# GAP-LAB-CUHK-SZ/REC-MV

Hardware: AMD Instinct MI355X
Metric: optimiser iters/sec, female-3-casual-like 512x512 (synthetic frames) (higher is better)
Workload: dtype f32

## Files before the change

rec-mv_amd/csrc/gemm_f32.hip:

```cpp
#include <mutex>
#include <unordered_map>
#include <type_traits>
#include <vector>
#include "common.h"
#ifdef RECMV_LIBM_SOFTPLUS
#define RECMV_EXPF(x) expf(x)
#define RECMV_LOG1PF(t) log1pf(t)
#else
#define RECMV_EXPF(x) __expf(x)
#define RECMV_LOG1PF(t) __logf(1.f + (t))
#endif

#include <algorithm>

namespace recmv {
namespace {

typedef float f32x16 __attribute__((ext_vector_type(16)));
typedef float f32x2 __attribute__((ext_vector_type(2)));
typedef __bf16 bf16x2 __attribute__((ext_vector_type(2)));
typedef __bf16 bf16x8 __attribute__((ext_vector_type(8)));
typedef unsigned int u32x4 __attribute__((ext_vector_type(4)));

struct Pieces {
  bf16x8 h, m, l;
};
__device__ __forceinline__ unsigned pack_bf16(float a, float b) {
#ifdef RECMV_SPLIT_INT
  unsigned ua = __float_as_uint(a), ub = __float_as_uint(b);
  ua += 0x7fffu + ((ua >> 16) & 1u);
  ub += 0x7fffu + ((ub >> 16) & 1u);
  return (ua >> 16) | (ub & 0xffff0000u);
#else
// ... 292 lines not shown
    }
    if (kt + 1 < nk) lstore(buf ^ 1);
    __syncthreads();
  }

  constexpr int LDC = TBN + 4;
  float* Cs = smem;
#pragma unroll
  for (int mi = 0; mi < T; ++mi)
#pragma unroll
    for (int ni = 0; ni < T; ++ni)
#pragma unroll
      for (int r = 0; r < 16; ++r) {
        const int row = wm * WT + mi * 32 + (r & 3) + 8 * (r >> 2) + 4 * (lane >> 5);
        const int col = wn * WT + ni * 32 + (lane & 31);
        Cs[row * LDC + col] = acc[mi][ni][r];
      }
  __syncthreads();
  switch (act) {
    case RECMV_ACT_RELU:
      nt_epilogue<T, RECMV_ACT_RELU>(Cs, bias, C, ldc, M, N, m0, n0, act_param, out_scale, c_vec, AMUL ? AMul{nullptr, 0, 0, 0.f, 1.f, 1.f} : am);
      break;
    case RECMV_ACT_SOFTPLUS:
      nt_epilogue<T, RECMV_ACT_SOFTPLUS>(Cs, bias, C, ldc, M, N, m0, n0, act_param, out_scale, c_vec, AMUL ? AMul{nullptr, 0, 0, 0.f, 1.f, 1.f} : am);
      break;
    case RECMV_ACT_TANH:
      nt_epilogue<T, RECMV_ACT_TANH>(Cs, bias, C, ldc, M, N, m0, n0, act_param, out_scale, c_vec, AMUL ? AMul{nullptr, 0, 0, 0.f, 1.f, 1.f} : am);
      break;
    default:
      nt_epilogue<T, RECMV_ACT_NONE>(Cs, bias, C, ldc, M, N, m0, n0, act_param, out_scale, c_vec, AMUL ? AMul{nullptr, 0, 0, 0.f, 1.f, 1.f} : am);
  }
}

template <bool AMUL, int BKT, bool SINGLE, int MI, int NI>
__global__ __launch_bounds__(kBlk, (MI * NI == 4 ? (BKT <= 16 ? 4 : 3) : 5))
void gemm_nt_occ_kernel(const float* __restrict__ A, int64_t lda, const float* __restrict__ B, int64_t ldb,
                        const float* __restrict__ bias, float* __restrict__ C, int64_t ldc, int M, int N, int K, int act,
                        float act_param, float out_scale, int nbm, int nbn, bool c_vec, AMul am) {
  constexpr int TBM = 64 * MI, TBN = 64 * NI;
  constexpr int LDKT = BKT + 4;
  constexpr int C4R = BKT / 4;
  constexpr int NLA = TBM * C4R / kBlk, NLB = TBN * C4R / kBlk;
  constexpr int NBUF = SINGLE ? 1 : 2;
  extern __shared__ __attribute__((aligned(16))) float smem[];
  float* As = smem;
  float* Bs = smem + NBUF * TBM * LDKT;
  const int tid = threadIdx.x, lane = tid & 63, wave = tid >> 6;
  const int wm = wave >> 1, wn = wave & 1;
  const int64_t logical = xcd_remap(blockIdx.x, (int64_t)nbm * nbn);
  const int tile_m = (int)(logical / nbn), tile_n = (int)(logical % nbn);
  const int m0 = tile_m * TBM, n0 = tile_n * TBN;
  if (am.B2 && m0 >= am.split) {
    B = am.B2;
    bias = am.bias2;
  }
  f32x16 acc[MI][NI];
#pragma unroll
  for (int a = 0; a < MI; ++a)
#pragma unroll
    for (int b = 0; b < NI; ++b)
#pragma unroll
      for (int r = 0; r < 16; ++r) acc[a][b][r] = 0.f;

  float4 ra[NLA], rb[NLB];
  const float* pa[NLA];
  const float* pb[NLB];
  const float* py[NLA];
#pragma unroll
  for (int r = 0; r < NLA; ++r) {
    const int idx = tid + kBlk * r;
    int gm = m0 + idx / C4R;
    gm = gm < M ? gm : M - 1;
    pa[r] = A + (int64_t)gm * lda + (idx % C4R) * 4;
    if (AMUL) py[r] = am.Y + (int64_t)gm * am.ldy + (idx % C4R) * 4;
  }
#pragma unroll
  for (int r = 0; r < NLB; ++r) {
    const int idx = tid + kBlk * r;
    int gn = n0 + idx / C4R;
    gn = gn < N ? gn : N - 1;
    pb[r] = B + (int64_t)gn * ldb + (idx % C4R) * 4;
  }
  auto gload = [&](int k0) {
#pragma unroll
    for (int r = 0; r < NLA; ++r) {
      const bool in = k0 + ((tid + kBlk * r) % C4R) * 4 < K;
      ra[r] = in ? *reinterpret_cast<const float4*>(pa[r] + k0) : make_float4(0, 0, 0, 0);
      if (AMUL && in) ra[r] = amul4(ra[r], *reinterpret_cast<const float4*>(py[r] + k0), am);
    }
#pragma unroll
    for (int r = 0; r < NLB; ++r) {
      const bool in = k0 + ((tid + kBlk * r) % C4R) * 4 < K;
      rb[r] = in ? *reinterpret_cast<const float4*>(pb[r] + k0) : make_float4(0, 0, 0, 0);
    }
  };
  auto lstore = [&](int buf) {
#pragma unroll
    for (int r = 0; r < NLA; ++r) {
      const int idx = tid + kBlk * r;
      *reinterpret_cast<float4*>(As + (buf * TBM + idx / C4R) * LDKT + (idx % C4R) * 4) = ra[r];
    }
#pragma unroll
    for (int r = 0; r < NLB; ++r) {
      const int idx = tid + kBlk * r;
      *reinterpret_cast<float4*>(Bs + (buf * TBN + idx / C4R) * LDKT + (idx % C4R) * 4) = rb[r];
    }
  };

  const int nk = (K + BKT - 1) / BKT;
  gload(0);
  lstore(0);
  __syncthreads();
  const int arow = wm * 32 * MI + (lane & 31), brow = wn * 32 * NI + (lane & 31), khalf = (lane >> 5) * 4;
  for (int kt = 0; kt < nk; ++kt) {
    const int buf = SINGLE ? 0 : (kt & 1);
    if (kt + 1 < nk) gload((kt + 1) * BKT);
    const float* as = As + (buf * TBM + arow) * LDKT + khalf;
    const float* bs = Bs + (buf * TBN + brow) * LDKT + khalf;
#pragma unroll
    for (int kk = 0; kk < BKT / 8; ++kk) {
      float4 a[MI], b[NI];
#pragma unroll
      for (int i = 0; i < MI; ++i) a[i] = *reinterpret_cast<const float4*>(as + i * 32 * LDKT + kk * 8);
#pragma unroll
      for (int i = 0; i < NI; ++i) b[i] = *reinterpret_cast<const float4*>(bs + i * 32 * LDKT + kk * 8);
// ... 14 lines not shown

  constexpr int HR = 32 * MI, LDC = TBN + 4;
  float* Cs = smem;
  const AMul em = AMUL ? AMul{nullptr, 0, 0, 0.f, 1.f, 1.f} : am;
#pragma unroll 1
  for (int h = 0; h < 2; ++h) {
    if (h) __syncthreads();
    if (wm == h) {
#pragma unroll
      for (int mi = 0; mi < MI; ++mi)
#pragma unroll
        for (int ni = 0; ni < NI; ++ni)
#pragma unroll
          for (int r = 0; r < 16; ++r) {
            const int row = mi * 32 + (r & 3) + 8 * (r >> 2) + 4 * (lane >> 5);
            const int col = wn * 32 * NI + ni * 32 + (lane & 31);
            Cs[row * LDC + col] = acc[mi][ni][r];
          }
    }
    __syncthreads();
    const int mh = m0 + HR * h;
    switch (act) {
      case RECMV_ACT_RELU:
        nt_epilogue_rows<HR, TBN, RECMV_ACT_RELU>(Cs, bias, C, ldc, M, N, mh, n0, act_param, out_scale, c_vec, em);
        break;
      case RECMV_ACT_SOFTPLUS:
        nt_epilogue_rows<HR, TBN, RECMV_ACT_SOFTPLUS>(Cs, bias, C, ldc, M, N, mh, n0, act_param, out_scale, c_vec, em);
        break;
      case RECMV_ACT_TANH:
        nt_epilogue_rows<HR, TBN, RECMV_ACT_TANH>(Cs, bias, C, ldc, M, N, mh, n0, act_param, out_scale, c_vec, em);
        break;
      default:
        nt_epilogue_rows<HR, TBN, RECMV_ACT_NONE>(Cs, bias, C, ldc, M, N, mh, n0, act_param, out_scale, c_vec, em);
    }
  }
}

__device__ __forceinline__ int b3_off(int row, int chunk) { return row * 64 + ((chunk ^ ((row >> 2) & 3)) << 4); }

struct B3Pre {
  const char* planes;
  const char* planes2;
  int64_t plane_bytes, plane_bytes2;
  int Kp;
};

template <int T, bool AMUL, bool PRE>
__global__ __launch_bounds__(kBlk, 2) void gemm_nt_b3_kernel(const float* __restrict__ A, int64_t lda,
                                                             const float* __restrict__ B, int64_t ldb,
                                                             const float* __restrict__ bias, float* __restrict__ C,
                                                             int64_t ldc, int M, int N, int K, int act,
                                                             float act_param, float out_scale, int nbm, int nbn,
                                                             bool c_vec, AMul am, B3Pre pre) {
  constexpr int TBM = 64 * T, TBN = 64 * T, WT = 32 * T;
  constexpr int NI = TBM * 4 / kBlk;
  constexpr int PLANE = TBM * 64;
  constexpr int NSET = 1;
  extern __shared__ __attribute__((aligned(16))) float smem[];
  char* As = reinterpret_cast<char*>(smem);
  char* Bs = As + 3 * PLANE;
  const int tid = threadIdx.x, lane = tid & 63, wave = tid >> 6;
  const int wm = wave >> 1, wn = wave & 1;
  const int64_t logical = xcd_remap(blockIdx.x, (int64_t)nbm * nbn);
  const int tile_m = (int)(logical / nbn), tile_n = (int)(logical % nbn);
  const int m0 = tile_m * TBM, n0 = tile_n * TBN;
  const char* planes = pre.planes;
// ... 533 lines not shown
    } else {
    const float* as = As + (buf * BK + kh) * LDM + acol;
    const float* bs = Bs + (buf * BK + kh) * LDM + bcol;
#pragma unroll
    for (int k2 = 0; k2 < BK / 2; ++k2) {
      const float a0 = as[k2 * 2 * LDM], a1 = as[k2 * 2 * LDM + 32];
      const float b0 = bs[k2 * 2 * LDM], b1 = bs[k2 * 2 * LDM + 32];
      acc[0][0] = __builtin_amdgcn_mfma_f32_32x32x2f32(a0, b0, acc[0][0], 0, 0, 0);
      acc[0][1] = __builtin_amdgcn_mfma_f32_32x32x2f32(a0, b1, acc[0][1], 0, 0, 0);
      acc[1][0] = __builtin_amdgcn_mfma_f32_32x32x2f32(a1, b0, acc[1][0], 0, 0, 0);
      acc[1][1] = __builtin_amdgcn_mfma_f32_32x32x2f32(a1, b1, acc[1][1], 0, 0, 0);
    }
    }
    if (kt + 1 < nk) lstore(buf ^ 1);
    __syncthreads();
  }

  float* Ps = P + (int64_t)split * M * N;
#pragma unroll
  for (int ni = 0; ni < 2; ++ni) {
    const int gn = n0 + wn * 64 + ni * 32 + (lane & 31);
    if (gn >= N) continue;
#pragma unroll
    for (int mi = 0; mi < 2; ++mi) {
#pragma unroll
      for (int r = 0; r < 16; ++r) {
        const int gm = m0 + wm * 64 + mi * 32 + (r & 3) + 8 * (r >> 2) + 4 * (lane >> 5);
        if (gm < M) Ps[(int64_t)gm * N + gn] = acc[mi][ni][r];
      }
    }
  }
}

template <int BKT>
__global__ __launch_bounds__(kBlk, 4) void gemm_tn_occ_kernel(const float* __restrict__ A, int64_t lda,
                                                              const float* __restrict__ B, int64_t ldb,
                                                              float* __restrict__ P, int M, int N, int64_t K, int nbm,
                                                              int nbn, int64_t kchunk) {
  constexpr int NLD = BKT * 32 / kBlk;
  extern __shared__ __attribute__((aligned(16))) float smem[];
  float* As = smem;
  float* Bs = smem + BKT * LDM;
  const int tid = threadIdx.x, lane = tid & 63, wave = tid >> 6;
  const int wm = wave >> 1, wn = wave & 1;
  const int tiles = nbm * nbn;
  int split = blockIdx.x / tiles, tile = blockIdx.x % tiles;
  const int splits = gridDim.x / tiles;
  if (splits % kNumXCD == 0) {
    const int x = blockIdx.x % kNumXCD, j = blockIdx.x / kNumXCD;
    split = x + kNumXCD * (j / tiles);
    tile = j % tiles;
  }
  const int tile_m = tile / nbn, tile_n = tile % nbn;
  const int m0 = tile_m * BM, n0 = tile_n * BN;
  const int64_t kbeg = (int64_t)split * kchunk;
  int64_t kend = kbeg + kchunk;
  if (kend > K) kend = K;

  f32x16 acc[2][2];
#pragma unroll
  for (int a = 0; a < 2; ++a)
#pragma unroll
    for (int b = 0; b < 2; ++b)
#pragma unroll
      for (int r = 0; r < 16; ++r) acc[a][b][r] = 0.f;

  float4 ra[NLD], rb[NLD];
  const bool whole_mn = m0 + BM <= M && n0 + BN <= N;
  auto gload = [&](int64_t k0) {
    const bool whole = whole_mn && k0 + BKT <= kend;
#pragma unroll
    for (int r = 0; r < NLD; ++r) {
      const int idx = tid + kBlk * r;
      const int krow = idx >> 5, c4 = idx & 31;
      const int64_t k = k0 + krow;
      const int cm = m0 + c4 * 4, cn = n0 + c4 * 4;
      if (whole) {
        ra[r] = *reinterpret_cast<const float4*>(A + k * lda + cm);
        rb[r] = *reinterpret_cast<const float4*>(B + k * ldb + cn);
      } else {
        const bool kin = k < kend, ain = kin && cm < M, bin = kin && cn < N;
        const int64_t kc = kin ? k : kend - 1;
        float4 a = *reinterpret_cast<const float4*>(A + kc * lda + (cm < M ? cm : (M - 1) & ~3));
        float4 b = *reinterpret_cast<const float4*>(B + kc * ldb + (cn < N ? cn : (N - 1) & ~3));
        ra[r] = make_float4(ain ? a.x : 0.f, ain ? a.y : 0.f, ain ? a.z : 0.f, ain ? a.w : 0.f);
        rb[r] = make_float4(bin ? b.x : 0.f, bin ? b.y : 0.f, bin ? b.z : 0.f, bin ? b.w : 0.f);
      }
    }
  };
  auto lstore = [&]() {
#pragma unroll
    for (int r = 0; r < NLD; ++r) {
      const int idx = tid + kBlk * r;
      const int krow = idx >> 5, c4 = idx & 31;
      *reinterpret_cast<float4*>(As + krow * LDM + c4 * 4) = ra[r];
      *reinterpret_cast<float4*>(Bs + krow * LDM + c4 * 4) = rb[r];
    }
  };

  const int nk = (int)((kend - kbeg + BKT - 1) / BKT);
  if (nk > 0) {
    gload(kbeg);
    lstore();
  }
  __syncthreads();
  const int acol = wm * 64 + (lane & 31), bcol = wn * 64 + (lane & 31), kh = lane >> 5;
  const float* as = As + kh * LDM + acol;
  const float* bs = Bs + kh * LDM + bcol;
  for (int kt = 0; kt < nk; ++kt) {
    if (kt + 1 < nk) gload(kbeg + (int64_t)(kt + 1) * BKT);
#pragma unroll
    for (int k2 = 0; k2 < BKT / 2; ++k2) {
      const float a0 = as[k2 * 2 * LDM], a1 = as[k2 * 2 * LDM + 32];
      const float b0 = bs[k2 * 2 * LDM], b1 = bs[k2 * 2 * LDM + 32];
      acc[0][0] = __builtin_amdgcn_mfma_f32_32x32x2f32(a0, b0, acc[0][0], 0, 0, 0);
      acc[0][1] = __builtin_amdgcn_mfma_f32_32x32x2f32(a0, b1, acc[0][1], 0, 0, 0);
      acc[1][0] = __builtin_amdgcn_mfma_f32_32x32x2f32(a1, b0, acc[1][0], 0, 0, 0);
      acc[1][1] = __builtin_amdgcn_mfma_f32_32x32x2f32(a1, b1, acc[1][1], 0, 0, 0);
    }
    __syncthreads();
    if (kt + 1 < nk) lstore();
    __syncthreads();
  }

  float* Ps = P + (int64_t)split * M * N;
#pragma unroll
  for (int ni = 0; ni < 2; ++ni) {
    const int gn = n0 + wn * 64 + ni * 32 + (lane & 31);
    if (gn >= N) continue;
#pragma unroll
    for (int mi = 0; mi < 2; ++mi) {
#pragma unroll
      for (int r = 0; r < 16; ++r) {
        const int gm = m0 + wm * 64 + mi * 32 + (r & 3) + 8 * (r >> 2) + 4 * (lane >> 5);
        if (gm < M) Ps[(int64_t)gm * N + gn] = acc[mi][ni][r];
      }
    }
  }
}

__global__ __launch_bounds__(kBlk) void splitk_reduce_kernel(const float* __restrict__ P, float* __restrict__ C,
                                                             int64_t ldc, int M, int N, int splits) {
  const int64_t total = (int64_t)M * N;
  for (int64_t i = (int64_t)blockIdx.x * kBlk + threadIdx.x; i < total; i += (int64_t)gridDim.x * kBlk) {
    float s = 0.f;
    for (int sp = 0; sp < splits; ++sp) s += P[(int64_t)sp * total + i];
    C[(i / N) * ldc + (i % N)] = s;
  }
}

__global__ __launch_bounds__(kBlk) void splitk_reduce4_kernel(const float4* __restrict__ P, float* __restrict__ C,
                                                              int64_t ldc, int M, int N, int splits) {
  const int64_t total4 = (int64_t)M * N / 4;
  for (int64_t i = (int64_t)blockIdx.x * kBlk + threadIdx.x; i < total4; i += (int64_t)gridDim.x * kBlk) {
    float4 s = make_float4(0.f, 0.f, 0.f, 0.f);
    int sp = 0;
    for (; sp + 8 <= splits; sp += 8) {
      float4 v[8];
#pragma unroll
      for (int u = 0; u < 8; ++u) v[u] = P[(int64_t)(sp + u) * total4 + i];
#pragma unroll
      for (int u = 0; u < 8; ++u) {
        s.x += v[u].x;
        s.y += v[u].y;
        s.z += v[u].z;
        s.w += v[u].w;
      }
    }
    for (; sp < splits; ++sp) {
      const float4 v = P[(int64_t)sp * total4 + i];
      s.x += v.x;
// ... 78 lines not shown
    if (!active) return;
    const double flops = 2.0 * M * N * K;
    r.bytes = 4.0 * (M * K + N * K + M * N);
    if (flops < g_prof.min_flops) {
      std::lock_guard<std::mutex> lk(g_prof.mu);
      g_prof.untimed[variant][0] += 1.0;
      g_prof.untimed[variant][1] += flops;
      active = false;
      return;
    }
    r.variant = variant;
    r.flops = flops;
    r.a = g_prof.get();
    r.b = g_prof.get();
    if (!r.a || !r.b) {
      active = false;
      return;
    }
    (void)hipEventRecord(r.a, s);
  }
  ~ScopedLaunchTimer() {
    if (!active) return;
    (void)hipEventRecord(r.b, s);
    std::lock_guard<std::mutex> lk(g_prof.mu);
    g_prof.recs.push_back(r);
  }
};

inline bool aligned16(const void* p) { return (reinterpret_cast<uintptr_t>(p) & 15) == 0; }

constexpr int kNtLds = (2 * BM * LDK + 2 * BN * LDK) * 4;
constexpr int kTnLds = (4 * BK * LDM) * 4;

bool tn_occ() {
  static const bool v = [] { const char* e = getenv("RECMV_GEMM_OCC"); return !(e && e[0] == '0'); }();
  return v;
}

int tn_splits(int64_t M, int64_t N, int64_t K) {
  const int64_t tiles = ceil_div(M, BM) * ceil_div(N, BN);
  int64_t want = ceil_div((int64_t)kNumCU * 4, tiles);
  const int64_t maxs = ceil_div(K, (int64_t)BK * 4);
  if (want > maxs) want = maxs;
  if (want > 128) want = 128;
  if (want < 1) want = 1;
  return (int)want;
}

}
}

using namespace recmv;

int g_b3_families = 7;
int g_gemm_mode = 0;

template <int T, bool FAST, bool AMUL, bool BF3>
static int launch_nt(const float* A, int64_t lda, const float* B, int64_t ldb, const float* bias, float* C,
                     int64_t ldc, int64_t M, int64_t N, int64_t K, int act, float act_param, float out_scale,
                     bool a_vec, bool b_vec, bool c_vec, const AMul& am, hipStream_t stream) {
  constexpr int lds = kNtLds / (T == 2 ? 1 : 2);
  static bool attr_set = false;
  if (!attr_set) {
    RECMV_HIP_TRY(hipFuncSetAttribute((const void*)gemm_nt_kernel<T, FAST, AMUL, BF3>,
                                      hipFuncAttributeMaxDynamicSharedMemorySize, lds));
    attr_set = true;
  }
  const int nbm = (int)ceil_div(M, 64 * T), nbn = (int)ceil_div(N, 64 * T);
  ScopedLaunchTimer timer((T - 1) + 2 * (FAST ? 1 : 0) + 4 * (AMUL ? 1 : 0), (double)M, (double)N, (double)K, stream);
  hipLaunchKernelGGL((gemm_nt_kernel<T, FAST, AMUL, BF3>), dim3((unsigned)((int64_t)nbm * nbn)), dim3(kBlk), lds, stream, A,
                     lda, B, ldb, bias, C, ldc, (int)M, (int)N, (int)K, act, act_param, out_scale, nbm, nbn, a_vec,
                     b_vec, c_vec, am);
  return check_launch("gemm_nt");
}

template <bool AMUL, int BKT, bool SINGLE, int MI, int NI>
static int launch_nt_occ(const float* A, int64_t lda, const float* B, int64_t ldb, const float* bias, float* C,
                         int64_t ldc, int64_t M, int64_t N, int64_t K, int act, float act_param, float out_scale,
                         bool c_vec, const AMul& am, hipStream_t stream) {
  constexpr int lds_ops = (SINGLE ? 1 : 2) * 64 * (MI + NI) * (BKT + 4) * 4, lds_c = 32 * MI * (64 * NI + 4) * 4;
  constexpr int lds = lds_ops > lds_c ? lds_ops : lds_c;
  const int nbm = (int)ceil_div(M, 64 * MI), nbn = (int)ceil_div(N, 64 * NI);
  ScopedLaunchTimer timer(AMUL ? 11 : (MI == 2 ? 9 : 10), (double)M, (double)N, (double)K, stream);
  hipLaunchKernelGGL((gemm_nt_occ_kernel<AMUL, BKT, SINGLE, MI, NI>), dim3((unsigned)((int64_t)nbm * nbn)), dim3(kBlk), lds,
                     stream, A, lda, B, ldb, bias, C, ldc, (int)M, (int)N, (int)K, act, act_param, out_scale, nbm, nbn, c_vec,
                     am);
  return check_launch("gemm_nt(occ)");
}

struct B3Entry {
  const char* planes;
  int64_t N, K, ldb, Kp;
};
static std::mutex g_b3_mu;
static std::unordered_map<const float*, B3Entry> g_b3;
static bool b3_lookup(const float* B, int64_t N, int64_t K, int64_t ldb, B3Entry* out) {
  std::lock_guard<std::mutex> lock(g_b3_mu);
  auto it = g_b3.find(B);
  if (it == g_b3.end() || it->second.K != K || it->second.ldb != ldb || it->second.N < N) return false;
  *out = it->second;
  return true;
}

template <int T, bool AMUL, bool PRE>
static int launch_nt_b3_as(const float* A, int64_t lda, const float* B, int64_t ldb, const float* bias, float* C, int64_t ldc,
                           int64_t M, int64_t N, int64_t K, int act, float act_param, float out_scale, bool c_vec, const AMul& am,
                           const B3Pre& pre, hipStream_t stream) {
  constexpr int lds_ops = 6 * 64 * T * 64, lds_c = 64 * T * (64 * T + 4) * 4;
  constexpr int lds = lds_ops > lds_c ? lds_ops : lds_c;
  static bool attr_set = false;
  if (!attr_set) {
    RECMV_HIP_TRY(hipFuncSetAttribute((const void*)gemm_nt_b3_kernel<T, AMUL, PRE>,
                                      hipFuncAttributeMaxDynamicSharedMemorySize, lds));
    attr_set = true;
  }
  const int nbm = (int)ceil_div(M, 64 * T), nbn = (int)ceil_div(N, 64 * T);
  ScopedLaunchTimer timer((T - 1) + 2 + 4 * (AMUL ? 1 : 0), (double)M, (double)N, (double)K, stream);
  hipLaunchKernelGGL((gemm_nt_b3_kernel<T, AMUL, PRE>), dim3((unsigned)((int64_t)nbm * nbn)), dim3(kBlk), lds, stream, A, lda,
                     B, ldb, bias, C, ldc, (int)M, (int)N, (int)K, act, act_param, out_scale, nbm, nbn, c_vec, am, pre);
  return check_launch("gemm_nt(b3)");
// ... 6 lines not shown
  B3Entry e, e2;
  if (b3_lookup(B, N, K, ldb, &e) && (!am.B2 || (b3_lookup(am.B2, N, K, ldb, &e2) && e2.Kp == e.Kp))) {
    B3Pre pre = {e.planes, am.B2 ? e2.planes : nullptr, e.N * e.Kp * 2, am.B2 ? e2.N * e2.Kp * 2 : 0, (int)e.Kp};
    return launch_nt_b3_as<T, AMUL, true>(A, lda, B, ldb, bias, C, ldc, M, N, K, act, act_param, out_scale, c_vec, am, pre, stream);
  }
  B3Pre none = {nullptr, nullptr, 0, 0, 0};
  return launch_nt_b3_as<T, AMUL, false>(A, lda, B, ldb, bias, C, ldc, M, N, K, act, act_param, out_scale, c_vec, am, none, stream);
}

constexpr int kNarrowLds = 2 * (64 + 32) * LDK * 4;

template <bool FAST, bool AMUL, bool BF3>
static int launch_nt_narrow(const float* A, int64_t lda, const float* B, int64_t ldb, const float* bias, float* C,
                            int64_t ldc, int64_t M, int64_t N, int64_t K, int act, float act_param, float out_scale,
                            bool a_vec, bool b_vec, bool c_vec, const AMul& am, hipStream_t stream) {
  const int nbm = (int)ceil_div(M, 64), nbn = (int)ceil_div(N, 32);
  ScopedLaunchTimer timer(FAST && !AMUL ? 12 : 13, (double)M, (double)N, (double)K, stream);
  hipLaunchKernelGGL((gemm_nt_narrow_kernel<FAST, AMUL, BF3>), dim3((unsigned)((int64_t)nbm * nbn)), dim3(kBlk),
                     kNarrowLds, stream, A, lda, B, ldb, bias, C, ldc, (int)M, (int)N, (int)K, act, act_param, out_scale,
                     nbm, nbn, a_vec, b_vec, c_vec, am);
  return check_launch("gemm_nt(narrow)");
}

template <bool AMUL>
static int dispatch_nt(const float* A, int64_t lda, const float* B, int64_t ldb, const float* bias, float* C,
                       int64_t ldc, int64_t M, int64_t N, int64_t K, int act, float act_param, float out_scale,
                       const AMul& am, hipStream_t s) {
  const bool a_vec = aligned16(A) && lda % 4 == 0 && (!AMUL || (aligned16(am.Y) && am.ldy % 4 == 0));
  const bool b_vec = aligned16(B) && ldb % 4 == 0 && (!am.B2 || aligned16(am.B2));
  const bool c_vec = aligned16(C) && ldc % 4 == 0;
  const bool fast = a_vec && b_vec && K % 4 == 0 && K > 0;
  const int64_t big_blocks = ceil_div(M, BM) * ceil_div(N, BN);
  const bool bf3_big = g_gemm_mode == 1 && (g_b3_families & 1), bf3_mid = g_gemm_mode == 1 && (g_b3_families & 2);
#define RECMV_NT(TT, FF)                                                                                          \
  ((TT == 2 ? bf3_big : bf3_mid) ? launch_nt<TT, FF, AMUL, true>(A, lda, B, ldb, bias, C, ldc, M, N, K, act, act_param, out_scale, \
                                                    a_vec, b_vec, c_vec, am, s)                                    \
                    : launch_nt<TT, FF, AMUL, false>(A, lda, B, ldb, bias, C, ldc, M, N, K, act, act_param,        \
                                                     out_scale, a_vec, b_vec, c_vec, am, s))
  if (big_blocks >= 2 * kNumCU) {
    if (bf3_big && fast) {
      return launch_nt_b3<2, AMUL>(A, lda, B, ldb, bias, C, ldc, M, N, K, act, act_param, out_scale, c_vec, am, s);
    }
    static const bool occ = [] { const char* e = getenv("RECMV_GEMM_OCC"); return !(e && e[0] == '0'); }();
    if (fast && !bf3_big && occ) {
      if (big_blocks >= 3600)
        return launch_nt_occ<AMUL, 16, true, 2, 2>(A, lda, B, ldb, bias, C, ldc, M, N, K, act, act_param, out_scale, c_vec, am, s);
      return launch_nt_occ<AMUL, 16, true, 1, 2>(A, lda, B, ldb, bias, C, ldc, M, N, K, act, act_param, out_scale, c_vec, am, s);
    }
    return fast ? RECMV_NT(2, true) : RECMV_NT(2, false);
  }
  const int64_t mid_blocks = ceil_div(M, 64) * ceil_div(N, 64);
  if (mid_blocks < (5 * kNumCU) / 2) {
#define RECMV_NTN(FF)                                                                                                  \
  (bf3_mid ? launch_nt_narrow<FF, AMUL, true>(A, lda, B, ldb, bias, C, ldc, M, N, K, act, act_param, out_scale, \
                                                       a_vec, b_vec, c_vec, am, s)                                     \
                    : launch_nt_narrow<FF, AMUL, false>(A, lda, B, ldb, bias, C, ldc, M, N, K, act, act_param,          \
                                                        out_scale, a_vec, b_vec, c_vec, am, s))
    return fast ? RECMV_NTN(true) : RECMV_NTN(false);
#undef RECMV_NTN
  }
  return fast ? RECMV_NT(1, true) : RECMV_NT(1, false);
#undef RECMV_NT
}

extern "C" int recmv_set_gemm_mode(int mode) {
  const int prev = g_gemm_mode;
  if (mode == 0 || mode == 1) g_gemm_mode = mode;
  return prev;
}

extern "C" int recmv_get_gemm_mode(void) { return g_gemm_mode; }

extern "C" int recmv_set_b3_families(int mask) {
  const int prev = g_b3_families;
  if (mask >= 0 && mask <= 7) g_b3_families = mask;
  return prev;
}

extern "C" int64_t recmv_b3_planes_bytes(int64_t N, int64_t K) {
  if (N <= 0 || K <= 0) return 0;
  return 3 * N * (ceil_div(K, (int64_t)BK) * BK) * 2;
// ... 104 lines not shown
                             void* stream) {
  RECMV_REQUIRE(M >= 0 && N >= 0 && K >= 0, "gemm_tn: negative size");
  if (M == 0 || N == 0) return RECMV_OK;
  RECMV_REQUIRE(M < (1 << 20) && N < (1 << 20), "gemm_tn: output too large");
  hipStream_t s = (hipStream_t)stream;
  if (K == 0) {
    RECMV_REQUIRE(C && ldc >= N, "gemm_tn: bad output");
    for (int64_t m = 0; m < M; ++m) RECMV_HIP_TRY(hipMemsetAsync(C + m * ldc, 0, N * 4, s));
    return RECMV_OK;
  }
  RECMV_REQUIRE(A && B && C, "gemm_tn: NULL pointer");
  RECMV_REQUIRE(lda >= M && ldb >= N && ldc >= N, "gemm_tn: leading dimension too small");
  const int splits = tn_splits(M, N, K);
  const int64_t need = (int64_t)splits * M * N * 4;
  if (!workspace || workspace_bytes < need) {
    set_error("gemm_tn: workspace %lld < %lld bytes", (long long)workspace_bytes, (long long)need);
    return RECMV_ERR_WORKSPACE;
  }
  static bool attr_set = false;
  if (!attr_set) {
    RECMV_HIP_TRY(hipFuncSetAttribute((const void*)gemm_tn_kernel<false>, hipFuncAttributeMaxDynamicSharedMemorySize,
                                      kTnLds));
    RECMV_HIP_TRY(hipFuncSetAttribute((const void*)gemm_tn_kernel<true>, hipFuncAttributeMaxDynamicSharedMemorySize,
                                      kTnLds));
    attr_set = true;
  }
  const int nbm = (int)ceil_div(M, BM), nbn = (int)ceil_div(N, BN);
  int64_t kchunk = ceil_div(ceil_div(K, splits), BK) * BK;
  const bool a_vec = aligned16(A) && lda % 4 == 0, b_vec = aligned16(B) && ldb % 4 == 0;
  int rc;
  {
  ScopedLaunchTimer timer(8, (double)M, (double)N, (double)K, s);
  const bool bf3_tn = g_gemm_mode == 1 && (g_b3_families & 4);
  if (!bf3_tn && tn_occ() && a_vec && b_vec && lda >= ((M + 3) & ~3ll) && ldb >= ((N + 3) & ~3ll) && M >= 4 && N >= 4) {
    kchunk = ceil_div(ceil_div(K, splits), 16) * 16;
    hipLaunchKernelGGL(gemm_tn_occ_kernel<16>, dim3((unsigned)(nbm * nbn * splits)), dim3(kBlk), 2 * 16 * LDM * 4, s, A, lda,
                       B, ldb, (float*)workspace, (int)M, (int)N, K, nbm, nbn, kchunk);
  } else if (bf3_tn)
    hipLaunchKernelGGL(gemm_tn_kernel<true>, dim3((unsigned)(nbm * nbn * splits)), dim3(kBlk), kTnLds, s, A, lda, B,
                       ldb, (float*)workspace, (int)M, (int)N, K, nbm, nbn, kchunk, a_vec, b_vec);
  else
    hipLaunchKernelGGL(gemm_tn_kernel<false>, dim3((unsigned)(nbm * nbn * splits)), dim3(kBlk), kTnLds, s, A, lda, B,
                       ldb, (float*)workspace, (int)M, (int)N, K, nbm, nbn, kchunk, a_vec, b_vec);
  rc = check_launch("gemm_tn");
  }
  if (rc) return rc;
  if (N % 4 == 0 && ldc % 4 == 0 && aligned16(C) && aligned16(workspace))
    hipLaunchKernelGGL(splitk_reduce4_kernel, dim3(stream_grid(M * N / 4, kBlk)), dim3(kBlk), 0, s,
                       (const float4*)workspace, C, ldc, (int)M, (int)N, splits);
  else
    hipLaunchKernelGGL(splitk_reduce_kernel, dim3(stream_grid(M * N, kBlk)), dim3(kBlk), 0, s,
                       (const float*)workspace, C, ldc, (int)M, (int)N, splits);
  return check_launch("gemm_tn/reduce");
}

extern "C" int recmv_posenc_forward(const float* x, int64_t ldx, float* out, int64_t ldo, int64_t ldo_fill,
                                    int64_t P, int L, const float* weights_host, float out_scale,
                                    void* stream) {
  RECMV_REQUIRE(P >= 0 && L >= 0 && L <= 16, "posenc: bad size (P=%lld, L=%d)", (long long)P, L);
  if (P == 0) return RECMV_OK;
  RECMV_REQUIRE(x && out, "posenc: NULL pointer");
  RECMV_REQUIRE(ldx >= 3 && ldo >= 3 + 6 * L && ldo_fill <= ldo, "posenc: leading dimension too small");
  hipStream_t s = (hipStream_t)stream;
  PeWeights hw;
  for (int i = 0; i < 32; ++i) hw.w[i] = (weights_host && i < 2 * L) ? weights_host[i] : 1.f;
  hipLaunchKernelGGL(posenc_kernel, dim3(stream_grid(P * (1 + 2 * L), kBlk)), dim3(kBlk), 0, s, x, ldx, out, ldo,
                     ldo_fill, P, L, hw, out_scale);
  return check_launch("posenc");
}

extern "C" int recmv_profile_begin(double min_flops) {
  g_prof.recs.clear();
  for (auto& u : g_prof.untimed) u[0] = u[1] = 0.0;
  g_prof.min_flops = min_flops;
  g_prof.on = true;
  return RECMV_OK;
// ... 82 lines not shown
```

Measured before the change: 10.33.

## Add skinny GEMM routes for thin N, thin K, and unaligned operands

Adds dedicated kernels for NT GEMMs with K<=4 or N<=4 and for TN GEMMs with an output dimension <=4. Also adds an unaligned-operand variant of the occupancy NT and TN kernels that uses dword-aligned vector loads instead of falling back to the generic kernel. The aim is to stop small-dimension and misaligned shapes from wasting large MFMA tiles, and to let them use the faster occupancy paths. These routes are on by default behind environment switches, and a shape-logging helper is added. This adds more template instantiations and new edge-case handling for partial vectors.

```diff
diff --git a/rec-mv_amd/csrc/gemm_f32.hip b/rec-mv_amd/csrc/gemm_f32.hip
--- a/rec-mv_amd/csrc/gemm_f32.hip
+++ b/rec-mv_amd/csrc/gemm_f32.hip
@@ -1,4 +1,5 @@
 #include <mutex>
+#include <string>
 #include <unordered_map>
 #include <type_traits>
 #include <vector>
@@ -357,11 +358,24 @@
   }
 }
 
-template <bool AMUL, int BKT, bool SINGLE, int MI, int NI>
+typedef float f32x4_a4 __attribute__((ext_vector_type(4), aligned(4)));
+__device__ __forceinline__ float4 load4_dword(const float* __restrict__ p, int limit) {
+  if (limit >= 4) {
+    const f32x4_a4 v = *reinterpret_cast<const f32x4_a4*>(p);
+    return make_float4(v.x, v.y, v.z, v.w);
+  }
+  return load4_guard(p, limit, false);
+}
+
+__device__ __forceinline__ float4 keep4(float4 v, int limit) {
+  return make_float4(limit > 0 ? v.x : 0.f, limit > 1 ? v.y : 0.f, limit > 2 ? v.z : 0.f, limit > 3 ? v.w : 0.f);
+}
+
+template <bool AMUL, int BKT, bool SINGLE, int MI, int NI, bool SCAL = false>
 __global__ __launch_bounds__(kBlk, (MI * NI == 4 ? (BKT <= 16 ? 4 : 3) : 5))
 void gemm_nt_occ_kernel(const float* __restrict__ A, int64_t lda, const float* __restrict__ B, int64_t ldb,
                         const float* __restrict__ bias, float* __restrict__ C, int64_t ldc, int M, int N, int K, int act,
-                        float act_param, float out_scale, int nbm, int nbn, bool c_vec, AMul am) {
+                        float act_param, float out_scale, int nbm, int nbn, bool c_vec, AMul am, bool a_vec, bool b_vec) {
   constexpr int TBM = 64 * MI, TBN = 64 * NI;
   constexpr int LDKT = BKT + 4;
   constexpr int C4R = BKT / 4;
@@ -391,6 +405,7 @@
   const float* pa[NLA];
   const float* pb[NLB];
   const float* py[NLA];
+  bool va[NLA], vb[NLB];
 #pragma unroll
   for (int r = 0; r < NLA; ++r) {
     const int idx = tid + kBlk * r;
@@ -398,6 +413,7 @@
     gm = gm < M ? gm : M - 1;
     pa[r] = A + (int64_t)gm * lda + (idx % C4R) * 4;
     if (AMUL) py[r] = am.Y + (int64_t)gm * am.ldy + (idx % C4R) * 4;
+    va[r] = a_vec && gm < M - 1;
   }
 #pragma unroll
   for (int r = 0; r < NLB; ++r) {
@@ -405,17 +421,33 @@
     int gn = n0 + idx / C4R;
     gn = gn < N ? gn : N - 1;
     pb[r] = B + (int64_t)gn * ldb + (idx % C4R) * 4;
+    vb[r] = b_vec && gn < N - 1;
   }
   auto gload = [&](int k0) {
 #pragma unroll
     for (int r = 0; r < NLA; ++r) {
-      const bool in = k0 + ((tid + kBlk * r) % C4R) * 4 < K;
+      const int k = k0 + ((tid + kBlk * r) % C4R) * 4;
+      if (SCAL) {
+        ra[r] = va[r] ? keep4(k < K ? *reinterpret_cast<const float4*>(pa[r] + k0) : make_float4(0, 0, 0, 0), K - k)
+                      : load4_dword(pa[r] + k0, K - k);
+        if (AMUL && k < K)
+          ra[r] = amul4(ra[r], va[r] ? keep4(*reinterpret_cast<const float4*>(py[r] + k0), K - k)
+                                     : load4_dword(py[r] + k0, K - k), am);
+        continue;
+      }
+      const bool in = k < K;
       ra[r] = in ? *reinterpret_cast<const float4*>(pa[r] + k0) : make_float4(0, 0, 0, 0);
       if (AMUL && in) ra[r] = amul4(ra[r], *reinterpret_cast<const float4*>(py[r] + k0), am);
     }
 #pragma unroll
     for (int r = 0; r < NLB; ++r) {
-      const bool in = k0 + ((tid + kBlk * r) % C4R) * 4 < K;
+      const int k = k0 + ((tid + kBlk * r) % C4R) * 4;
+      if (SCAL) {
+        rb[r] = vb[r] ? keep4(k < K ? *reinterpret_cast<const float4*>(pb[r] + k0) : make_float4(0, 0, 0, 0), K - k)
+                      : load4_dword(pb[r] + k0, K - k);
+        continue;
+      }
+      const bool in = k < K;
       rb[r] = in ? *reinterpret_cast<const float4*>(pb[r] + k0) : make_float4(0, 0, 0, 0);
     }
   };
@@ -496,6 +528,163 @@
         break;
       default:
         nt_epilogue_rows<HR, TBN, RECMV_ACT_NONE>(Cs, bias, C, ldc, M, N, mh, n0, act_param, out_scale, c_vec, em);
+    }
+  }
+}
+
+__device__ __forceinline__ float apply_act_rt(float z, int act, float p, float inv_p) {
+  switch (act) {
+    case RECMV_ACT_RELU: return apply_act<RECMV_ACT_RELU>(z, p, inv_p);
+    case RECMV_ACT_SOFTPLUS: return apply_act<RECMV_ACT_SOFTPLUS>(z, p, inv_p);
+    case RECMV_ACT_TANH: return apply_act<RECMV_ACT_TANH>(z, p, inv_p);
+    default: return z;
+  }
+}
+
+constexpr int kThinRows = 128;
+template <int NN, bool VEC>
+__global__ __launch_bounds__(kThinRows) void gemm_nt_thin_n_kernel(const float* __restrict__ A, int64_t lda,
+                                                                   const float* __restrict__ B, int64_t ldb,
+                                                                   const float* __restrict__ bias, float* __restrict__ C,
+                                                                   int64_t ldc, int M, int K, int act, float act_param,
+                                                                   float out_scale, bool halves, AMul am) {
+  __shared__ __attribute__((aligned(16))) float As[kThinRows * LDK];
+  __shared__ __attribute__((aligned(16))) float Bs[4 * LDK];
+  const int tid = threadIdx.x;
+  const int m0 = blockIdx.x * kThinRows;
+  if (am.B2 && m0 >= am.split) {
+    B = am.B2;
+    bias = am.bias2;
+  }
+  constexpr int NLD = kThinRows * 8 / kThinRows;
+  float4 ra[NLD];
+  float rb;
+  const float* pa[NLD];
+#pragma unroll
+  for (int r = 0; r < NLD; ++r) {
+    const int idx = tid + kThinRows * r;
+    int gm = m0 + (idx >> 3);
+    gm = gm < M ? gm : M - 1;
+    pa[r] = A + (int64_t)gm * lda + (idx & 7) * 4;
+  }
+  const int bn = tid >> 5, bk = tid & 31;
+  auto gload = [&](int k0) {
+#pragma unroll
+    for (int r = 0; r < NLD; ++r) {
+      const int k = k0 + ((tid + kThinRows * r) & 7) * 4;
+      if (VEC)
+        ra[r] = k < K ? *reinterpret_cast<const float4*>(pa[r] + k0) : make_float4(0, 0, 0, 0);
+      else
+        ra[r] = load4_dword(pa[r] + k0, K - k);
+    }
+    rb = (bn < NN && k0 + bk < K) ? B[(int64_t)bn * ldb + k0 + bk] : 0.f;
+  };
+  auto lstore = [&]() {
+#pragma unroll
+    for (int r = 0; r < NLD; ++r) {
+      const int idx = tid + kThinRows * r;
+      *reinterpret_cast<float4*>(As + (idx >> 3) * LDK + (idx & 7) * 4) = ra[r];
+    }
+    Bs[bn * LDK + bk] = rb;
+  };
+  float acc[2][NN];
+#pragma unroll
+  for (int n = 0; n < NN; ++n) acc[0][n] = acc[1][n] = 0.f;
+  const int nk = (K + BK - 1) / BK;
+  gload(0);
+  lstore();
+  __syncthreads();
+  const float* as = As + tid * LDK;
+  for (int kt = 0; kt < nk; ++kt) {
+    if (kt + 1 < nk) gload((kt + 1) * BK);
+#pragma unroll
+    for (int kk = 0; kk < BK / 8; ++kk) {
+      const float4 a0 = *reinterpret_cast<const float4*>(as + kk * 8);
+      const float4 a1 = *reinterpret_cast<const float4*>(as + kk * 8 + 4);
+#pragma unroll
+      for (int n = 0; n < NN; ++n) {
+        const float4 b0 = *reinterpret_cast<const float4*>(Bs + n * LDK + kk * 8);
+        const float4 b1 = *reinterpret_cast<const float4*>(Bs + n * LDK + kk * 8 + 4);
+        const int h = (halves && kk >= BK / 16) ? 1 : 0;
+        float s = acc[h][n];
+        s = fmaf(a0.x, b0.x, s);
+        s = fmaf(a1.x, b1.x, s);
+        s = fmaf(a0.y, b0.y, s);
+        s = fmaf(a1.y, b1.y, s);
+        s = fmaf(a0.z, b0.z, s);
+        s = fmaf(a1.z, b1.z, s);
+        s = fmaf(a0.w, b0.w, s);
+        s = fmaf(a1.w, b1.w, s);
+        acc[h][n] = s;
+      }
+    }
+    __syncthreads();
+    if (kt + 1 < nk) lstore();
+    __syncthreads();
+  }
+  const int gm = m0 + tid;
+  if (gm >= M) return;
+  const float inv_p = act_param != 0.f ? 1.f / act_param : 0.f;
+#pragma unroll
+  for (int n = 0; n < NN; ++n) {
+    const float z = halves ? acc[0][n] + acc[1][n] : acc[0][n];
+    float v = apply_act_rt(z + (bias ? bias[n] : 0.f), act, act_param, inv_p) * out_scale;
+    if (am.Y) v *= dact_y(am.Y[(int64_t)gm * am.ldy + n] * am.y_scale, am.act, am.param) * am.a_scale;
+    C[(int64_t)gm * ldc + n] = v;
+  }
+}
+
+constexpr int kThinKRows = 32;
+template <int KK, bool AMUL>
+__global__ __launch_bounds__(kBlk) void gemm_nt_thin_k_kernel(const float* __restrict__ A, int64_t lda,
+                                                              const float* __restrict__ B, int64_t ldb,
+                                                              const float* __restrict__ bias, float* __restrict__ C,
+                                                              int64_t ldc, int M, int N, int act, float act_param,
+                                                              float out_scale, int cw_log2, bool c_vec, AMul am) {
+  const int tid = threadIdx.x;
+  const int cw = 1 << cw_log2, cl = tid & (cw - 1), rsub = tid >> cw_log2, rstep = kBlk >> cw_log2;
+  const int m0 = blockIdx.x * kThinKRows;
+  const int mend = m0 + kThinKRows < M ? m0 + kThinKRows : M;
+  if (am.B2 && m0 >= am.split) {
+    B = am.B2;
+    bias = am.bias2;
+  }
+  const float inv_p = act_param != 0.f ? 1.f / act_param : 0.f;
+  for (int gn = cl * 4; gn < N; gn += cw * 4) {
+    float b[4][KK], bv[4];
+#pragma unroll
+    for (int j = 0; j < 4; ++j) {
+      bv[j] = (bias && gn + j < N) ? bias[gn + j] : 0.f;
+#pragma unroll
+      for (int k = 0; k < KK; ++k) b[j][k] = gn + j < N ? B[(int64_t)(gn + j) * ldb + k] : 0.f;
+    }
+    const bool full4 = c_vec && gn + 4 <= N;
+    for (int gm = m0 + rsub; gm < mend; gm += rstep) {
+      float a[KK];
+#pragma unroll
+      for (int k = 0; k < KK; ++k) {
+        a[k] = A[(int64_t)gm * lda + k];
+        if (AMUL) a[k] *= dact_y(am.Y[(int64_t)gm * am.ldy + k] * am.y_scale, am.act, am.param) * am.a_scale;
+      }
+      float o[4];
+#pragma unroll
+      for (int j = 0; j < 4; ++j) {
+        float s = 0.f;
+#pragma unroll
+        for (int k = 0; k < KK; ++k) s = fmaf(a[k], b[j][k], s);
+        o[j] = apply_act_rt(s + bv[j], act, act_param, inv_p) * out_scale;
+      }
+      float4 v = make_float4(o[0], o[1], o[2], o[3]);
+      if (!AMUL && am.Y) v = emul4(v, am, gm, gn, N);
+      float* dst = C + (int64_t)gm * ldc + gn;
+      if (full4) {
+        *reinterpret_cast<float4*>(dst) = v;
+      } else {
+        dst[0] = v.x;
+        if (gn + 1 < N) dst[1] = v.y;
+        if (gn + 2 < N) dst[2] = v.z;
+        if (gn + 3 < N) dst[3] = v.w;
+      }
     }
   }
 }
@@ -1095,7 +1284,7 @@
   }
 }
 
-template <int BKT>
+template <int BKT, bool SCAL = false>
 __global__ __launch_bounds__(kBlk, 4) void gemm_tn_occ_kernel(const float* __restrict__ A, int64_t lda,
                                                               const float* __restrict__ B, int64_t ldb,
                                                               float* __restrict__ P, int M, int N, int64_t K, int nbm,
@@ -1138,7 +1327,10 @@
       const int krow = idx >> 5, c4 = idx & 31;
       const int64_t k = k0 + krow;
       const int cm = m0 + c4 * 4, cn = n0 + c4 * 4;
-      if (whole) {
+      if (SCAL) {
+        ra[r] = k < kend ? load4_dword(A + k * lda + cm, M - cm) : make_float4(0, 0, 0, 0);
+        rb[r] = k < kend ? load4_dword(B + k * ldb + cn, N - cn) : make_float4(0, 0, 0, 0);
+      } else if (whole) {
         ra[r] = *reinterpret_cast<const float4*>(A + k * lda + cm);
         rb[r] = *reinterpret_cast<const float4*>(B + k * ldb + cn);
       } else {
@@ -1200,6 +1392,32 @@
       }
     }
   }
+}
+
+template <int NT, bool SWAP>
+__global__ __launch_bounds__(kWave) void gemm_tn_thin_kernel(const float* __restrict__ T, int64_t ldt,
+                                                             const float* __restrict__ W, int64_t ldw,
+                                                             float* __restrict__ P, int NW, int64_t K, int64_t kchunk,
+                                                             int ntile) {
+  const int tile = blockIdx.x % ntile, split = blockIdx.x / ntile;
+  const int c = tile * kWave + threadIdx.x;
+  if (c >= NW) return;
+  const int64_t kbeg = (int64_t)split * kchunk;
+  int64_t kend = kbeg + kchunk;
+  if (kend > K) kend = K;
+  float acc[NT];
+#pragma unroll
+  for (int t = 0; t < NT; ++t) acc[t] = 0.f;
+  const float* w = W + c;
+#pragma unroll 16
+  for (int64_t k = kbeg; k < kend; ++k) {
+    const float wv = w[k * ldw];
+#pragma unroll
+    for (int t = 0; t < NT; ++t) acc[t] = fmaf(T[k * ldt + t], wv, acc[t]);
+  }
+  float* Ps = P + (int64_t)split * NT * NW;
+#pragma unroll
+  for (int t = 0; t < NT; ++t) Ps[SWAP ? (int64_t)c * NT + t : (int64_t)t * NW + c] = acc[t];
 }
 
 __global__ __launch_bounds__(kBlk) void splitk_reduce_kernel(const float* __restrict__ P, float* __restrict__ C,
@@ -1344,6 +1562,11 @@
 constexpr int kNtLds = (2 * BM * LDK + 2 * BN * LDK) * 4;
 constexpr int kTnLds = (4 * BK * LDM) * 4;
 
+bool skinny_routes() {
+  const char* e = getenv("RECMV_GEMM_SKINNY");
+  return !(e && e[0] == '0');
+}
+
 bool tn_occ() {
   static const bool v = [] { const char* e = getenv("RECMV_GEMM_OCC"); return !(e && e[0] == '0'); }();
   return v;
@@ -1386,18 +1609,71 @@
   return check_launch("gemm_nt");
 }
 
-template <bool AMUL, int BKT, bool SINGLE, int MI, int NI>
+template <bool AMUL, int BKT, bool SINGLE, int MI, int NI, bool SCAL = false>
 static int launch_nt_occ(const float* A, int64_t lda, const float* B, int64_t ldb, const float* bias, float* C,
                          int64_t ldc, int64_t M, int64_t N, int64_t K, int act, float act_param, float out_scale,
-                         bool c_vec, const AMul& am, hipStream_t stream) {
+                         bool c_vec, const AMul& am, hipStream_t stream, bool a_vec = true, bool b_vec = true) {
   constexpr int lds_ops = (SINGLE ? 1 : 2) * 64 * (MI + NI) * (BKT + 4) * 4, lds_c = 32 * MI * (64 * NI + 4) * 4;
   constexpr int lds = lds_ops > lds_c ? lds_ops : lds_c;
   const int nbm = (int)ceil_div(M, 64 * MI), nbn = (int)ceil_div(N, 64 * NI);
-  ScopedLaunchTimer timer(AMUL ? 11 : (MI == 2 ? 9 : 10), (double)M, (double)N, (double)K, stream);
-  hipLaunchKernelGGL((gemm_nt_occ_kernel<AMUL, BKT, SINGLE, MI, NI>), dim3((unsigned)((int64_t)nbm * nbn)), dim3(kBlk), lds,
+  ScopedLaunchTimer timer(SCAL ? (AMUL ? 5 : 1) : (AMUL ? 11 : (MI == 2 ? 9 : 10)), (double)M, (double)N, (double)K, stream);
+  hipLaunchKernelGGL((gemm_nt_occ_kernel<AMUL, BKT, SINGLE, MI, NI, SCAL>), dim3((unsigned)((int64_t)nbm * nbn)), dim3(kBlk), lds,
                      stream, A, lda, B, ldb, bias, C, ldc, (int)M, (int)N, (int)K, act, act_param, out_scale, nbm, nbn, c_vec,
-                     am);
+                     am, a_vec, b_vec);
   return check_launch("gemm_nt(occ)");
+}
+
+static int nt_old_slot(int64_t M, int64_t N, bool fast, bool amul) {
+  const int64_t big_blocks = ceil_div(M, BM) * ceil_div(N, BN);
+  if (big_blocks >= 2 * kNumCU) {
+    if (!fast) return amul ? 5 : 1;
+    return amul ? 11 : (big_blocks >= 3600 ? 9 : 10);
+  }
+  if (ceil_div(M, 64) * ceil_div(N, 64) < (5 * kNumCU) / 2) return fast && !amul ? 12 : 13;
+  return 2 * (fast ? 1 : 0) + 4 * (amul ? 1 : 0);
+}
+
+template <int NN>
+static int launch_nt_thin_n(const float* A, int64_t lda, const float* B, int64_t ldb, const float* bias, float* C,
+                            int64_t ldc, int64_t M, int64_t K, int act, float act_param, float out_scale, bool vec,
+                            const AMul& am, int slot, hipStream_t stream) {
+  ScopedLaunchTimer timer(slot, (double)M, (double)NN, (double)K, stream);
+  const dim3 grid((unsigned)ceil_div(M, kThinRows));
+  const bool halves = ceil_div(M, 64) < (5 * kNumCU) / 2;
+  if (vec)
+    hipLaunchKernelGGL((gemm_nt_thin_n_kernel<NN, true>), grid, dim3(kThinRows), 0, stream, A, lda, B, ldb, bias, C, ldc, (int)M,
+                       (int)K, act, act_param, out_scale, halves, am);
+  else
+    hipLaunchKernelGGL((gemm_nt_thin_n_kernel<NN, false>), grid, dim3(kThinRows), 0, stream, A, lda, B, ldb, bias, C, ldc, (int)M,
+                       (int)K, act, act_param, out_scale, halves, am);
+  return check_launch("gemm_nt(thin n)");
+}
+
+template <int KK, bool AMUL>
+static int launch_nt_thin_k(const float* A, int64_t lda, const float* B, int64_t ldb, const float* bias, float* C,
+                            int64_t ldc, int64_t M, int64_t N, int act, float act_param, float out_scale, bool c_vec,
+                            const AMul& am, int slot, hipStream_t stream) {
+  ScopedLaunchTimer timer(slot, (double)M, (double)N, (double)KK, stream);
+  int cw_log2 = 0;
+  while (cw_log2 < 8 && (4ll << cw_log2) < N) ++cw_log2;
+  hipLaunchKernelGGL((gemm_nt_thin_k_kernel<KK, AMUL>), dim3((unsigned)ceil_div(M, kThinKRows)), dim3(kBlk), 0, stream, A, lda, B,
+                     ldb, bias, C, ldc, (int)M, (int)N, act, act_param, out_scale, cw_log2, c_vec, am);
+  return check_launch("gemm_nt(thin k)");
+}
+
+static void log_shape(const char* route, const char* parent, int64_t M, int64_t N, int64_t K, int64_t lda, int64_t ldb, const void* A, const void* B,
+                      bool amul, bool emul, bool seg) {
+  static const bool on = [] { const char* e = getenv("RECMV_GEMM_SHAPES"); return e && e[0] == '1'; }();
+  if (!on || (double)M * (double)N * (double)K < 1e8) return;
+  static std::mutex mu;
+  static std::unordered_map<std::string, int> seen;
+  char key[256];
+  snprintf(key, sizeof key, "%s (before: %s) M=%lld N=%lld K=%lld lda=%lld ldb=%lld A%%16=%d B%%16=%d amul=%d emul=%d seg=%d", route, parent,
+           (long long)M,
+           (long long)N, (long long)K, (long long)lda, (long long)ldb, (int)(reinterpret_cast<uintptr_t>(A) & 15),
+           (int)(reinterpret_cast<uintptr_t>(B) & 15), (int)amul, (int)emul, (int)seg);
+  std::lock_guard<std::mutex> lk(mu);
+  if (seen[key]++ == 0) fprintf(stderr, "[recmv shapes] %s\n", key);
 }
 
 struct B3Entry {
@@ -1470,7 +1746,37 @@
   const bool fast = a_vec && b_vec && K % 4 == 0 && K > 0;
   const int64_t big_blocks = ceil_div(M, BM) * ceil_div(N, BN);
   const bool bf3_big = g_gemm_mode == 1 && (g_b3_families & 1), bf3_mid = g_gemm_mode == 1 && (g_b3_families & 2);
-#define RECMV_NT(TT, FF)                                                                                          \
+  static const bool occ_env = [] { const char* e = getenv("RECMV_GEMM_OCC"); return !(e && e[0] == '0'); }();
+  const bool occ = occ_env, skinny = occ_env && skinny_routes();
+  const char* parent_route = big_blocks >= 2 * kNumCU ? (fast ? "nt_occ" : "nt_kernel<2,false>") : "below 512 large tiles";
+  if (g_gemm_mode == 0 && skinny && K >= 1 && K <= 4) {
+    const int slot = nt_old_slot(M, N, fast, AMUL);
+    log_shape("thin_k", parent_route, M, N, K, lda, ldb, A, B, AMUL, !AMUL && am.Y, am.B2 != nullptr);
+#define RECMV_TK(KK) \
+  case KK: return launch_nt_thin_k<KK, AMUL>(A, lda, B, ldb, bias, C, ldc, M, N, act, act_param, out_scale, c_vec, am, slot, s)
+    switch (K) {
+      RECMV_TK(1);
+      RECMV_TK(2);
+      RECMV_TK(3);
+      default: RECMV_TK(4);
+    }
+#undef RECMV_TK
+  }
+  if (g_gemm_mode == 0 && skinny && !AMUL && N <= 4) {
+    const int slot = nt_old_slot(M, N, fast, false);
+    const bool vec = a_vec && K % 4 == 0;
+    log_shape("thin_n", parent_route, M, N, K, lda, ldb, A, B, false, am.Y != nullptr, am.B2 != nullptr);
+#define RECMV_TN_(NN) \
+  case NN: return launch_nt_thin_n<NN>(A, lda, B, ldb, bias, C, ldc, M, K, act, act_param, out_scale, vec, am, slot, s)
+    switch (N) {
+      RECMV_TN_(1);
+      RECMV_TN_(2);
+      RECMV_TN_(3);
+      default: RECMV_TN_(4);
+    }
+#undef RECMV_TN_
+  }
+#define RECMV_NT(TT, FF)                                                                                         \
   ((TT == 2 ? bf3_big : bf3_mid) ? launch_nt<TT, FF, AMUL, true>(A, lda, B, ldb, bias, C, ldc, M, N, K, act, act_param, out_scale, \
                                                     a_vec, b_vec, c_vec, am, s)                                    \
                     : launch_nt<TT, FF, AMUL, false>(A, lda, B, ldb, bias, C, ldc, M, N, K, act, act_param,        \
@@ -1479,12 +1785,18 @@
     if (bf3_big && fast) {
       return launch_nt_b3<2, AMUL>(A, lda, B, ldb, bias, C, ldc, M, N, K, act, act_param, out_scale, c_vec, am, s);
     }
-    static const bool occ = [] { const char* e = getenv("RECMV_GEMM_OCC"); return !(e && e[0] == '0'); }();
     if (fast && !bf3_big && occ) {
       if (big_blocks >= 3600)
         return launch_nt_occ<AMUL, 16, true, 2, 2>(A, lda, B, ldb, bias, C, ldc, M, N, K, act, act_param, out_scale, c_vec, am, s);
       return launch_nt_occ<AMUL, 16, true, 1, 2>(A, lda, B, ldb, bias, C, ldc, M, N, K, act, act_param, out_scale, c_vec, am, s);
     }
+    if (!fast && !bf3_big && skinny && K > 0) {
+      log_shape("occ_scal", parent_route, M, N, K, lda, ldb, A, B, AMUL, !AMUL && am.Y, am.B2 != nullptr);
+      if (big_blocks >= 3600)
+        return launch_nt_occ<AMUL, 16, true, 2, 2, true>(A, lda, B, ldb, bias, C, ldc, M, N, K, act, act_param, out_scale, c_vec, am, s, a_vec && lda >= K, b_vec);
+      return launch_nt_occ<AMUL, 16, true, 1, 2, true>(A, lda, B, ldb, bias, C, ldc, M, N, K, act, act_param, out_scale, c_vec, am, s, a_vec && lda >= K, b_vec);
+    }
+    if (!fast) log_shape("nt_kernel<2,false>", parent_route, M, N, K, lda, ldb, A, B, AMUL, !AMUL && am.Y, am.B2 != nullptr);
     return fast ? RECMV_NT(2, true) : RECMV_NT(2, false);
   }
   const int64_t mid_blocks = ceil_div(M, 64) * ceil_div(N, 64);
@@ -1655,16 +1967,44 @@
   {
   ScopedLaunchTimer timer(8, (double)M, (double)N, (double)K, s);
   const bool bf3_tn = g_gemm_mode == 1 && (g_b3_families & 4);
-  if (!bf3_tn && tn_occ() && a_vec && b_vec && lda >= ((M + 3) & ~3ll) && ldb >= ((N + 3) & ~3ll) && M >= 4 && N >= 4) {
+  if (!bf3_tn && tn_occ() && skinny_routes() && (M <= 4 || N <= 4)) {
+    const bool swap = M > 4;
+    const float* T = swap ? B : A;
+    const float* W = swap ? A : B;
+    const int64_t ldt = swap ? ldb : lda, ldw = swap ? lda : ldb, NT = swap ? N : M, NW = swap ? M : N;
+    const bool was_occ = a_vec && b_vec && lda >= ((M + 3) & ~3ll) && ldb >= ((N + 3) & ~3ll) && M >= 4 && N >= 4;
+    kchunk = ceil_div(ceil_div(K, splits), was_occ ? 16 : BK) * (was_occ ? 16 : BK);
+    const int ntile = (int)ceil_div(NW, kWave);
+    const dim3 grid((unsigned)((int64_t)ntile * splits));
+    log_shape("tn_thin", was_occ ? "tn_occ" : "tn_kernel<false>", M, N, K, lda, ldb, A, B, false, false, false);
+#define RECMV_TT(NTT, SW) \
+  hipLaunchKernelGGL((gemm_tn_thin_kernel<NTT, SW>), grid, dim3(kWave), 0, s, T, ldt, W, ldw, (float*)workspace, (int)NW, K, kchunk, ntile)
+#define RECMV_TT2(NTT) \
+  case NTT: if (swap) RECMV_TT(NTT, true); else RECMV_TT(NTT, false); break
+    switch (NT) {
+      RECMV_TT2(1);
+      RECMV_TT2(2);
+      RECMV_TT2(3);
+      default: RECMV_TT2(4);
+    }
+#undef RECMV_TT2
+#undef RECMV_TT
+  } else if (!bf3_tn && tn_occ() && a_vec && b_vec && lda >= ((M + 3) & ~3ll) && ldb >= ((N + 3) & ~3ll) && M >= 4 && N >= 4) {
     kchunk = ceil_div(ceil_div(K, splits), 16) * 16;
     hipLaunchKernelGGL(gemm_tn_occ_kernel<16>, dim3((unsigned)(nbm * nbn * splits)), dim3(kBlk), 2 * 16 * LDM * 4, s, A, lda,
+                       B, ldb, (float*)workspace, (int)M, (int)N, K, nbm, nbn, kchunk);
+  } else if (!bf3_tn && tn_occ() && skinny_routes() && M > 4 && N > 4) {
+    log_shape("tn_occ_scal", "tn_kernel<false>", M, N, K, lda, ldb, A, B, false, false, false);
+    hipLaunchKernelGGL((gemm_tn_occ_kernel<16, true>), dim3((unsigned)(nbm * nbn * splits)), dim3(kBlk), 2 * 16 * LDM * 4, s, A, lda,
                        B, ldb, (float*)workspace, (int)M, (int)N, K, nbm, nbn, kchunk);
   } else if (bf3_tn)
     hipLaunchKernelGGL(gemm_tn_kernel<true>, dim3((unsigned)(nbm * nbn * splits)), dim3(kBlk), kTnLds, s, A, lda, B,
                        ldb, (float*)workspace, (int)M, (int)N, K, nbm, nbn, kchunk, a_vec, b_vec);
-  else
+  else {
+    log_shape("tn_kernel<false>", "tn_kernel<false>", M, N, K, lda, ldb, A, B, false, false, false);
     hipLaunchKernelGGL(gemm_tn_kernel<false>, dim3((unsigned)(nbm * nbn * splits)), dim3(kBlk), kTnLds, s, A, lda, B,
                        ldb, (float*)workspace, (int)M, (int)N, K, nbm, nbn, kchunk, a_vec, b_vec);
+  }
   rc = check_launch("gemm_tn");
   }
   if (rc) return rc;
```

Result: faster. 10.53 (median of 6 runs) (+1.9%).
